# lukeshope/hipims-ocl

Measured on AMD Instinct MI355X. Metric: Mcell-steps/sec fp64 Godunov+HLLC, 4096^2 grid, 1/2/4/8 MI355X; % HBM roofline, higher is better.
Workload: dtype f64

## Files before the change

### hipims-ocl_amd/csrc/hp_domain.hpp

```cpp
#pragma once
#include "../../include/hipims_mi.h"
#include "hp_facts.hpp"
#include "hp_kernels.hpp"
#include "hp_peaks.hpp"
#include "hp_probes.hpp"
#include "hp_zones.hpp"
#include "hp_overview.hpp"
#include "hp_sparse.hpp"
#include "hp_bed.hpp"
#include <rccl/rccl.h>

#include <atomic>
#include <string>
#include <vector>

using namespace hp;

namespace {

thread_local std::string g_last_error;

std::atomic<hp_log_sink_t> g_log_sink{nullptr};
std::atomic<void*>         g_log_user{nullptr};

// ... 130 lines not shown
	void*            saved_scalars = nullptr;
	bool             saved_valid = false;
	ncclComm_t       comm = nullptr;
	int              comm_rank = 0, comm_world = 1;
	hipEvent_t       ev_xchg = nullptr;
	unsigned long long*  peer_mine = nullptr;
	unsigned long long** peer_table = nullptr;
	std::vector<void*>   peer_mapped;
	int              peer_world = 0, peer_rank = 0;
	bool             peer_agreed = false;
	uint64_t         peer_rounds = 0;
	void*            peer_state[2][2] = {{nullptr, nullptr}, {nullptr, nullptr}};
	long             peer_rows[2] = {0, 0};
	unsigned*        push_arrived = nullptr;
	bool             peer_direct = false;
	bool             push_now = false;
	unsigned long long* tail_words = nullptr;
	bool             fill_now = false;
	void*            z_state = nullptr;
	unsigned long long* haz_words = nullptr;
	unsigned         pair_gen = 0;
	void*            still_rec = nullptr;
	size_t           still_rec_slots = 0;
	int              still_rec_half = 0;
	bool             still_rec_last = false;
	uint64_t         pair_cold_starts = 0;
	hipEvent_t       tune_ev[4] = {nullptr, nullptr, nullptr, nullptr};
	int              tune_phase = 0;
	bool             tune_prefer_pairs = true;
	uint64_t         tune_next = 0;
	uint64_t         tune_samples = 0, tune_switches = 0;
	float            tune_pair_ms = 0.f, tune_single_ms = 0.f;
	uint64_t         pairs = 0;
	unsigned         single_streak = 0;
	uint64_t         flux_launches = 0, flux_launches_tailed = 0;
	bool             tail_failed = false;
	bool             strip_first = false;
	bool             tail_allowed = false;
	bool             tail_want = false;
	int              tail_fresh = 0;
	bool             tail_done = false;
	bool             spec_now = false;
	uint32_t         spec_pending = 0;
	void*            spec_state = nullptr;
	void*            spec_scalars = nullptr;
	struct { int adv_fresh; uint64_t cells_calculated, iterations; } spec_host;
	uint64_t         spec_batches = 0, spec_replays = 0;
	OutputStage      out;
// ... 30 lines not shown
```

### hipims-ocl_amd/csrc/hp_engine.hip

```cpp
#include "hp_domain.hpp"
#include "hp_observers.hpp"
#include <hip/hip_ext.h>
#include <dlfcn.h>

#include <algorithm>
#include <cmath>
#include <cstdio>
#include <cstdlib>
#include <cstring>
#include <random>
#include <string>
#include <vector>
#include <unistd.h>

namespace {

constexpr size_t CFL_SLOT_BYTES = 1024;

struct Rccl {
	void* handle = nullptr;
	decltype(&ncclGetUniqueId)   GetUniqueId = nullptr;
	decltype(&ncclCommInitRank)  CommInitRank = nullptr;
	decltype(&ncclCommDestroy)   CommDestroy = nullptr;
	decltype(&ncclGroupStart)    GroupStart = nullptr;
// ... 576 lines not shown
{
	if (d->desc.math_mode == HP_MATH_STRICT) return true;
	static const int forced = std::getenv("HP_PAIR_EXACT") ? (std::atoi(std::getenv("HP_PAIR_EXACT")) != 0 ? 1 : 0) : -1;
	if (forced >= 0) return forced != 0;
	for (const Boundary& b : d->bdy)
		if ((b.kind == 0 && b.definition == HP_UNIFORM_LOSS_RATE) || (b.kind == 1 && b.definition == HP_GRIDDED_MASS_FLUX)) return true;
	return false;
}
static int pair_stamps_alloc(hp_domain* d)
{
	if (!pair_exact(d) || d->z_state) return HP_OK;
	const size_t rec = (size_t)4 * d->esize + 16;
	HIP_TRY(hipMalloc(&d->z_state, d->cells * rec));
	HIP_TRY(hipMalloc((void**)&d->haz_words, 64));
	HIP_TRY(hipMemsetAsync(d->z_state, 0, d->cells * rec, d->stream));
	HIP_TRY(hipMemsetAsync(d->haz_words, 0, 64, d->stream));
	return HP_OK;
}
static bool pair_skip_enabled()
{
	static const bool v = !(std::getenv("HP_PAIR_SKIP") && std::atoi(std::getenv("HP_PAIR_SKIP")) == 0);
	return v;
}
static int still_rec_alloc(hp_domain* d, const int windows)
{
	const size_t slots = (size_t)windows * (size_t)d->desc.rows;
	if (d->still_rec && d->still_rec_slots == slots) return HP_OK;
	hipFree(d->still_rec);
	d->still_rec = nullptr;
	d->facts.buffers_written_outside();
	const size_t bytes = (2 * slots + 1) * sizeof(StillRec);
	HIP_TRY(hipMalloc(&d->still_rec, bytes));
	HIP_TRY(hipMemsetAsync(d->still_rec, 0xff, bytes, d->stream));
	d->still_rec_slots = slots;
	return HP_OK;
}
template <typename T> int pair_cold_start(hp_domain* d)
{
	int rc;
	d->facts.buffers_written_outside();
	if ((rc = apply_boundaries<T>(d, d->state[0])) != HP_OK) return rc;
	if ((rc = launch_reduce<T>(d, d->state[0], d->own_lo, d->own_hi)) != HP_OK) return rc;
	hipLaunchKernelGGL((pair_cold_start_words<T>), dim3(1), dim3(1), 0, d->stream, (T*)d->cfl_slot);
	HIP_TRY(hipGetLastError());
	d->facts.cold_started();
	d->pair_cold_starts++;
	return HP_OK;
}
template <typename T> int run_pair_t(hp_domain* d, const bool strip, const bool followed)
{
	const Params<T> p = make_params<T>(d);
	TileMap tm;
	unsigned blocks;
	long lo, hi;
	if (strip) {
		const bool south = d->desc.row_offset > 0, north = d->desc.row_offset + d->desc.rows < d->desc.global_rows;
		lo = south ? d->ghost_rows : 1;
// ... 11 lines not shown
	const int kind = make_tail<T>(d, blocks, PART_ALL, d->stream, tail_limit(), tail);
	d->tail_want = false; d->tail_allowed = false; d->push_now = false;
	if (kind != (strip ? 2 : 1)) return HP_ERR_STATE;
	const bool bdy = !d->bdy.empty();
	int rc;
	if ((rc = pair_stamps_alloc(d)) != HP_OK) return rc;
	bool in_place = false;
	if (bdy && !d->facts->m1_valid) {
		if ((rc = pair_cold_start<T>(d)) != HP_OK) return rc;
		in_place = true;
	} else if (bdy) in_place = d->facts->pair_fused_next;
	tail.pair = bdy ? 2 : 1;
	tail.bdy_flag = bdy && followed ? 1 : 0;
	PairAux<T> aux{};
	const bool exact = pair_exact(d) && d->z_state != nullptr;
	if (exact) aux.stamps = StampBufs<T>{(char*)d->z_state, d->haz_words};
	aux.prev_gen = d->facts->other_stale ? d->pair_gen : 0u;
	aux.gen = ++d->pair_gen;
	if (aux.gen == 0) aux.gen = ++d->pair_gen;
	aux.list = (const AreaBdyList<T>*)d->fused_list; aux.fuse_next = bdy && followed ? 1 : 0; aux.in_place = in_place ? 1 : 0;
	aux.truncated = (d->desc.quirks & HP_QUIRK_BDY_TRUNCATED) != 0 ? 1 : 0;
	const bool recs = sizeof(T) == 8 && pair_skip_enabled() && !strip && !bdy && !exact && d->desc.math_mode != HP_MATH_STRICT && rseg2 <= 32;
	if (recs) {
		if ((rc = still_rec_alloc(d, tm.nstrips)) != HP_OK) return rc;
		StillRec* const base = (StillRec*)d->still_rec;
		aux.still_out = base + (size_t)(d->still_rec_half ^ 1) * d->still_rec_slots;
		aux.still_in = d->facts->still_rec_valid ? base + (size_t)d->still_rec_half * d->still_rec_slots : nullptr;
		aux.still_rows = d->desc.rows;
	}
	const void* src = d->state[0];
	void* dst = d->state[1];
	const bool sample = d->timing_stride > 0 && d->timing_used < d->timing_events.size() &&
	                    (d->timing_counter++ % (uint64_t)d->timing_stride) == 0;
	if (sample) HIP_TRY(hipEventRecord(d->timing_events[d->timing_used].first, d->stream));
#define HP_LAUNCH_K1B2(CFL_, BDY_, HZ_, TAIL_)                                                                                            \
	hipLaunchKernelGGL((godunov_march2<false, CFL_, BDY_, HZ_, TAIL_, T>), dim3(blocks), dim3(256), 0, d->stream, p, (const Scalars<T>*)d->scalars, \
	                   (const T*)d->bed, (const State4<T>*)src, (State4<T>*)dst, (const T*)d->manning, (T*)d->cfl_slot,                    \
	                   (const T*)d->cfl_slot + SLOT_EDGE, tm, tail, aux)
#define HP_LAUNCH_K1B(CFL_, BDY_, TAIL_) do { if (exact) HP_LAUNCH_K1B2(CFL_, BDY_, true, TAIL_); else HP_LAUNCH_K1B2(CFL_, BDY_, false, TAIL_); } while (0)
	if (d->desc.math_mode == HP_MATH_STRICT)
		hipLaunchKernelGGL((godunov_march2<true, 1, false, true, 1, T>), dim3(blocks), dim3(256), 0, d->stream, p, (const Scalars<T>*)d->scalars,
		                   (const T*)d->bed, (const State4<T>*)src, (State4<T>*)dst, (const T*)d->manning, (T*)d->cfl_slot,
		                   (const T*)d->cfl_slot + SLOT_EDGE, tm, tail, aux);
	else
	if (strip)    { if (d->desc.dynamic_dt) HP_LAUNCH_K1B2(1, false, false, 2); else HP_LAUNCH_K1B2(0, false, false, 2); }
	else if (bdy) HP_LAUNCH_K1B(1, true, 1);
	else          { if (d->desc.dynamic_dt) HP_LAUNCH_K1B(1, false, 1); else HP_LAUNCH_K1B(0, false, 1); }
#undef HP_LAUNCH_K1B
#undef HP_LAUNCH_K1B2
	d->facts.pair_queued(bdy, followed);
	HIP_TRY(hipGetLastError());
// ... 1747 lines not shown
	double total = 0.0;
	uint32_t n = 0;
	for (size_t i = 0; i < d->timing_used; ++i) {
		float ms = 0.f;
		HIP_TRY(hipEventElapsedTime(&ms, d->timing_events[i].first, d->timing_events[i].second));
		total += std::max(0.0, (double)ms - d->timing_overhead_ms);
		++n;
	}
	*avg_ms = n ? total / n : 0.0;
	*samples = n;
	return HP_OK;
}

int hp_pair_stats(hp_domain_t* d, uint64_t out[12])
{
	int rc = check_domain(d);
	if (rc != HP_OK) return rc;
	if (!out) return fail(HP_ERR_INVALID, "out == NULL");
	out[0] = d->pairs; out[1] = d->pair_cold_starts; out[2] = out[3] = 0;
	HIP_TRY(hipStreamSynchronize(d->stream));
	if (tuner_on(d) && (rc = tuner_poll(d)) != HP_OK) return rc;
	out[4] = d->tune_samples; out[5] = d->tune_switches; out[6] = d->tune_prefer_pairs ? 1 : 0;
	out[7] = d->tune_single_ms > 0.f ? (uint64_t)(1000.0 * d->tune_pair_ms / d->tune_single_ms) : 0;
	out[8] = out[9] = out[10] = out[11] = 0;
	if (d->still_rec && d->still_rec_last) {
		const StillRec* half = (const StillRec*)d->still_rec + (size_t)d->still_rec_half * d->still_rec_slots;
		unsigned long long* counts = (unsigned long long*)((StillRec*)d->still_rec + 2 * d->still_rec_slots);
		HIP_TRY(hipMemsetAsync(counts, 0, 16, d->stream));
		hipLaunchKernelGGL(still_rec_count, dim3(256), dim3(256), 0, d->stream, half, d->still_rec_slots, counts);
		HIP_TRY(hipGetLastError());
		unsigned long long host_counts[2] = {0, 0};
		HIP_TRY(hipMemcpyAsync(host_counts, counts, sizeof host_counts, hipMemcpyDeviceToHost, d->stream));
		HIP_TRY(hipStreamSynchronize(d->stream));
		out[9] = host_counts[0]; out[10] = host_counts[1];
	}
	if (d->haz_words) {
		unsigned long long used = 0;
		HIP_TRY(hipMemcpy(&used, d->haz_words + 2, sizeof used, hipMemcpyDeviceToHost));
		out[8] = used;
	}
	if (!d->z_state) return HP_OK;
	unsigned long long* counts = d->haz_words + 4;
	HIP_TRY(hipMemsetAsync(counts, 0, 16, d->stream));
	if (d->desc.precision == 8)
		hipLaunchKernelGGL((stamps_count<double>), dim3(1024), dim3(256), 0, d->stream, StampBufs<double>{(char*)d->z_state, d->haz_words}, d->pair_gen, d->cells, counts);
	else
		hipLaunchKernelGGL((stamps_count<float>), dim3(1024), dim3(256), 0, d->stream, StampBufs<float>{(char*)d->z_state, d->haz_words}, d->pair_gen, d->cells, counts);
	HIP_TRY(hipGetLastError());
	unsigned long long host_counts[2] = {0, 0};
	HIP_TRY(hipMemcpyAsync(host_counts, counts, sizeof host_counts, hipMemcpyDeviceToHost, d->stream));
	HIP_TRY(hipStreamSynchronize(d->stream));
	out[2] = host_counts[0]; out[3] = host_counts[1];
	return HP_OK;
}

int hp_launch_counts(hp_domain_t* d, uint64_t* flux_launches, uint64_t* with_tail)
{
	int rc = check_domain(d);
	if (rc != HP_OK) return rc;
	if (!flux_launches || !with_tail) return fail(HP_ERR_INVALID, "null argument");
	*flux_launches = d->flux_launches;
	*with_tail = d->flux_launches_tailed;
	return HP_OK;
}

int hp_kernel_timing_overhead(hp_domain_t* d, double* overhead_ms)
{
	int rc = check_domain(d);
	if (rc != HP_OK) return rc;
	if (!overhead_ms) return fail(HP_ERR_INVALID, "null argument");
	*overhead_ms = d->timing_overhead_ms;
	return HP_OK;
}

}
```

### hipims-ocl_amd/csrc/hp_kernels.hpp

```cpp
#pragma once

#include "hp_math.hpp"
#include "hp_tiling.hpp"

namespace hp {

template <bool STRICT, typename T>
__global__ __launch_bounds__(256) void godunov_basic(const Params<T> p, const Scalars<T>* __restrict__ sc,
                                                     const T* __restrict__ bed, const State4<T>* __restrict__ src,
                                                     State4<T>* __restrict__ dst, const T* __restrict__ manning,
                                                     const long y_lo, const long y_hi)
{
	const long x = (long)blockIdx.x * blockDim.x + threadIdx.x;
	const long y = (long)blockIdx.y * blockDim.y + threadIdx.y + y_lo;
	if (x >= p.cols - 1 || y >= y_hi || x <= 0) return;
	const size_t id = (size_t)y * p.cols + x;
	const T dt = sc->dt;

	if (dt <= T(0)) { dst[id] = src[id]; return; }

	const State4<T> c = src[id];
	const T zb = bed[id], n = manning[id];
	if (c.zmax <= T(-9999.0) || c.z == T(-9999.0)) { dst[id] = c; return; }

// ... 182 lines not shown
	if (threadIdx.x != 0) return;
	advance_body<UPDATE_ONLY>(p, sc, slot, fresh & 3);
}

template <typename T> struct LaunchTail {
	unsigned long long* done;
	unsigned            flux_blocks;
	int                 pair;
	unsigned long long* done1;
	int                 bdy_flag;
	unsigned            poll_blocks;
	unsigned long long  timeout;
	int                 fresh;
	Scalars<T>*         sc;
	T*                  slot;
	PeerBox             box;
	State4<T>*          peer_rows[2];
	int                 edge_rows[4];
};

#ifndef HP_TAIL_FORMAL_ORDER
#define HP_TAIL_FORMAL_ORDER 0
#endif
template <bool TWO = false, typename T>
__device__ __forceinline__ void tail_block_done(const LaunchTail<T>& tail, const T m, const int wave, const int lane, const long y0, const long y1, const T m1 = T(0))
{
	__shared__ T part[4];
	__shared__ T part1[4];
	const bool sends = (y0 < tail.edge_rows[1] && y1 > tail.edge_rows[0]) || (y0 < tail.edge_rows[3] && y1 > tail.edge_rows[2]);
	if (sends) asm volatile("s_waitcnt vmcnt(0)" ::: "memory");
	if (lane == 0) { part[wave] = m; if (TWO) part1[wave] = m1; }
	__syncthreads();
	bool block_sends = false;
	if (threadIdx.x == 0) {
		block_sends = sends;
		T b = part[0];
		for (int w = 1; w < 4; ++w) if (part[w] > b) b = part[w];
		if (TWO) {
			T b1 = part1[0];
			for (int w = 1; w < 4; ++w) if (part1[w] > b1) b1 = part1[w];
			__hip_atomic_store(tail.done1 + blockIdx.x, peer_bits(b1), __ATOMIC_RELAXED, __HIP_MEMORY_SCOPE_AGENT);
		}
#if HP_TAIL_FORMAL_ORDER
		if (block_sends) __hip_atomic_store(tail.done + blockIdx.x, peer_bits(b), __ATOMIC_RELEASE, __HIP_MEMORY_SCOPE_SYSTEM);
		else
#endif
		__hip_atomic_store(tail.done + blockIdx.x, peer_bits(b), __ATOMIC_RELAXED, __HIP_MEMORY_SCOPE_AGENT);
		(void)block_sends;
	}
}

#ifndef HP_TAIL_POLL_SLEEP
#define HP_TAIL_POLL_SLEEP 1
#endif
template <typename T>
__device__ __forceinline__ void launch_tail(const Params<T>& p, const LaunchTail<T>& tail)
{
	__shared__ T part[4];
// ... 172 lines not shown
}
__device__ __forceinline__ float first_lane(const float v) { return __int_as_float(__builtin_amdgcn_readfirstlane(__float_as_int(v))); }
__device__ __forceinline__ double first_lane(const double v)
{
	return __hiloint2double(__builtin_amdgcn_readfirstlane(__double2hiint(v)), __builtin_amdgcn_readfirstlane(__double2loint(v)));
}
__device__ __forceinline__ unsigned long long value_bits(const double v) { return (unsigned long long)__double_as_longlong(v); }
template <typename V> __device__ __forceinline__ V from_east(const V v) { return lane_move<DPP_WAVE_ROL1>(v); }
template <typename V> __device__ __forceinline__ V from_west(const V v) { return lane_move<DPP_WAVE_ROR1>(v); }

template <typename T> struct RowRegs { State4<T> c; T zb, n; };

template <typename T>
__device__ __forceinline__ Side<T> side_from_east(const Side<T>& s)
{
	Side<T> r;
	r.eta = from_east(s.eta); r.zb = from_east(s.zb);
	r.qx = from_east(s.qx);   r.qy = from_east(s.qy);
	r.u0 = from_east(s.u0);   r.v0 = from_east(s.v0);
	return r;
}


__device__ __forceinline__ bool tile_rows(const TileMap& tm, const int wave, long& strip, long& y0, long& y1)
{
	const unsigned band = blockIdx.x % (unsigned)tm.nbands, i = blockIdx.x / (unsigned)tm.nbands;
	const unsigned nbig_tiles = (unsigned)(tm.groups * tm.nbig);
	const long band_y0 = tm.y_begin + (long)band * tm.band_stride;
	const long band_y1 = (band_y0 + tm.band_rows < tm.y_end) ? (band_y0 + tm.band_rows) : tm.y_end;
	unsigned g;
	long h;
	if (i < nbig_tiles) {
		g = i % (unsigned)tm.groups;
		h = tm.rseg;
		y0 = band_y0 + (long)(i / (unsigned)tm.groups) * tm.rseg;
	} else {
		const unsigned j = i - nbig_tiles;
		g = j % (unsigned)tm.groups;
		h = tm.rseg_tail;
		y0 = band_y0 + (long)tm.nbig * tm.rseg + (long)(j / (unsigned)tm.groups) * tm.rseg_tail;
	}
	y1 = (y0 + h < band_y1) ? (y0 + h) : band_y1;
	strip = (long)g * 4 + wave;
	const bool any = y0 < band_y1 && strip < tm.nstrips;
	if (tm.flip) {
		const long top = band_y0 + (band_y1 - y1);
		y1 = band_y0 + (band_y1 - y0);
		y0 = top;
	}
	return any;
}

template <typename T> struct UniformBdy { const T* series; uint32_t entries; int definition; T interval, length; };
template <typename T> struct GriddedBdy {
	const T* grids; uint64_t entries, grows, gcols; int definition; T resolution, off_x, off_y, interval;
};

template <typename T>
__device__ __forceinline__ bool bdy_in_range(const Params<T>& p, const long x, const long gy, const bool truncated)
{
	if (x >= p.cols - 1 || gy >= p.global_rows - 1 || x <= 0 || gy <= 0) return false;
	if (truncated && (x >= (p.cols / 8) * 8 || gy >= (p.global_rows / 8) * 8)) return false;
	return true;
}

constexpr int AREA_BDY_MAX = 8;
template <typename T> struct AreaBdy {
	int kind;
	UniformBdy<T> u;
	GriddedBdy<T> g;
};
template <typename T> struct AreaBdyList { int count; AreaBdy<T> b[AREA_BDY_MAX]; };


constexpr int FUSED_BDY_MAX = 3;
template <typename T> struct FusedBdy {
	T    inc_lo, inc_hi;
	int  y_switch;
	int  mode;
};

template <typename T> constexpr unsigned stamp_rec() { return (unsigned)sizeof(State4<T>) + 16u; }
template <typename T> struct StampBufs { char* rec; unsigned long long* haz; };
template <typename T> __device__ __forceinline__ unsigned stamp_gen(const StampBufs<T>& b, const size_t id)
{
	return *reinterpret_cast<const unsigned*>(b.rec + id * stamp_rec<T>() + sizeof(State4<T>));
}
template <typename T> __device__ __forceinline__ State4<T> stamp_state(const StampBufs<T>& b, const size_t id)
{
	const T* v = reinterpret_cast<const T*>(b.rec + id * stamp_rec<T>());
	State4<T> c; c.z = v[0]; c.zmax = v[1]; c.qx = v[2]; c.qy = v[3];
	return c;
}
struct StillRec { unsigned long long z, b; unsigned tag, pad[3]; };
constexpr unsigned STILL_TAG_RUN = 1, STILL_TAG_SKIP = 2;
template <typename T> struct PairAux {
	StampBufs<T>          stamps;
	unsigned              gen, prev_gen;
	const AreaBdyList<T>* list;
	int                   fuse_next;
	int                   in_place;
	int                   truncated;
	StillRec*             still_out;
	const StillRec*       still_in;
	long                  still_rows;
};

#ifndef HP_K1_STRICT_WAVES
#define HP_K1_STRICT_WAVES 3
#endif
#ifndef HP_K1_FAST_WAVES
#define HP_K1_FAST_WAVES 3
#endif
#ifndef HP_K1_F32_WAVES
#define HP_K1_F32_WAVES 5
#endif
template <bool STRICT, typename T> constexpr int march_waves() { return sizeof(T) == 4 ? HP_K1_F32_WAVES : (STRICT ? HP_K1_STRICT_WAVES : HP_K1_FAST_WAVES); }

template <bool STRICT, typename T> constexpr int march_waves_max() { return sizeof(T) == 4 ? 8 : march_waves<STRICT, T>(); }
template <bool STRICT, int CFL_MODE, bool FUSED, int TAIL, typename T, bool SPEC = false>
__global__ __launch_bounds__(256) __attribute__((amdgpu_waves_per_eu(march_waves<STRICT, T>(), march_waves_max<STRICT, T>()))) void godunov_march(const Params<T> p, const Scalars<T>* sc,
                                                     const T* __restrict__ bed, const State4<T>* __restrict__ src,
                                                     State4<T>* __restrict__ dst, const T* __restrict__ manning,
                                                     T* cfl_slot, const T* __restrict__ edge_max,
                                                     const TileMap tm, const AreaBdyList<T>* __restrict__ fused_list,
                                                     const int fuse_next, const int flags, const LaunchTail<T> tail)
{
	if (TAIL != 0 && blockIdx.x >= tail.flux_blocks) {
		launch_tail(p, tail);
// ... 310 lines not shown
	}
	if (FUSED && blockIdx.x == 0 && wave == 0 && lane == 0) cfl_slot[SLOT_BDY] = fuse_flag ? T(1) : T(0);
	}
	if (TAIL != 0) tail_block_done(tail, wave_vmax, wave, lane, y0, y1);
}

template <typename T> struct RowU1 { State4<T> c; T zb; bool plain; };

template <bool STRICT, int CFL_MODE, bool BDY, bool HZ, int TAIL, typename T>
#ifndef HP_K1B_WAVES_MIN
#define HP_K1B_WAVES_MIN 3
#endif
#ifndef HP_K1B_F32_WAVES_MIN
#define HP_K1B_F32_WAVES_MIN 5
#endif
#ifndef HP_K1B_F32_WAVES_MAX
#define HP_K1B_F32_WAVES_MAX 5
#endif
__global__ __launch_bounds__(256) __attribute__((amdgpu_waves_per_eu(sizeof(T) == 4 ? (STRICT ? 3 : (HZ ? 4 : HP_K1B_F32_WAVES_MIN)) : (STRICT ? HP_K1B_STRICT_WAVES : HP_K1B_WAVES_MIN), sizeof(T) == 4 ? (STRICT ? 3 : HP_K1B_F32_WAVES_MAX) : (STRICT ? HP_K1B_STRICT_WAVES : 3)))) void godunov_march2(
	const Params<T> p, const Scalars<T>* sc, const T* __restrict__ bed, const State4<T>* __restrict__ src,
	State4<T>* __restrict__ dst, const T* __restrict__ manning, T* cfl_slot, const T* __restrict__ edge_max,
	const TileMap tm, const LaunchTail<T> tail, const PairAux<T> aux)
{
	if (TAIL != 0 && blockIdx.x >= tail.flux_blocks) {
		launch_tail(p, tail);
		return;
	}
	__shared__ T inc_tab[BDY ? 4 * 3 * FUSED_BDY_MAX * 2 * 64 : 1];
	const int lane = threadIdx.x & 63, wave = __builtin_amdgcn_readfirstlane((int)(threadIdx.x >> 6));
	long strip, y0, y1;
	T wave_vmax = T(0), wave_vmax1 = T(0);
	if (tile_rows(tm, wave, strip, y0, y1)) {

	const long x = strip * MARCH2_COLS - 1 + lane;
	const long xc = x < 0 ? 0 : (x < p.cols ? x : (p.cols - 1));
	const bool out_x = lane >= 2 && lane <= MARCH2_COLS + 1 && x <= p.cols - 2;
	const bool ring_x = x <= 0 || x >= p.cols - 1;
	const T vs = p.vs;
	const bool with_friction = p.friction != 0;
	const T inv_dx = STRICT ? p.inv_dx_pow2 : p.inv_dx;

	Scalars<T> s1 = *sc;
	const Scalars<T> s0 = s1;
	const T dt_a = s1.dt;
	advance_scalars(p, s1, p.dynamic_dt ? cfl_slot[BDY ? SLOT_M1 : SLOT_SAVED] : T(0));
	const T dt_b = s1.dt;
	const bool skip_a = dt_a <= T(0), skip_b = dt_b <= T(0);
	constexpr bool SCALAR_CONSTS = !STRICT && sizeof(T) == 8;
	constexpr bool HIDE = BDY || HZ;
	const StepConsts<T> ka{uniform_value<HIDE>(-(dt_a * p.inv_dx)), uniform_value<HIDE>(dt_a * gravity<T>()), SCALAR_CONSTS};
	const StepConsts<T> kb{uniform_value<HIDE>(-(dt_b * p.inv_dx)), uniform_value<HIDE>(dt_b * gravity<T>()), SCALAR_CONSTS};

	const long row_base = y0 - 2 < 0 ? 0 : y0 - 2, col_base = strip * MARCH2_COLS - 1 < 0 ? 0 : strip * MARCH2_COLS - 1;
	const size_t cell0 = (size_t)row_base * p.cols + (size_t)col_base;
	const size_t cells_left = (size_t)p.cols * p.rows - cell0;
// ... 97 lines not shown
					if (b.g.definition == 0) {
						inc_lo = rate_lo / T(3600000.0) * thj[j];
						inc_hi = rate_hi / T(3600000.0) * thj[j];
					} else {
						inc_lo = rate_lo / (p.dx * p.dx) * thj[j];
						inc_hi = rate_hi / (p.dx * p.dx) * thj[j];
					}
					ysw[k] = (int)(row_base + n_lo);
					mode = 2u;
				}
				if (mode == 3u) continue;
				tab[((j * FUSED_BDY_MAX + k) * 2 + 0) * 64 + lane] = inc_lo;
				tab[((j * FUSED_BDY_MAX + k) * 2 + 1) * 64 + lane] = inc_hi;
				modes = (modes & ~(3u << (2 * (j * FUSED_BDY_MAX + k)))) | (mode << (2 * (j * FUSED_BDY_MAX + k)));
				act |= 1u << j;
			}
		}
	}
	const bool fuse = BDY && aux.fuse_next != 0;

	T vmax = T(0), vmax1 = T(0);
	unsigned stale_rows = 0;

	constexpr bool RECS = !STRICT && !BDY && !HZ && TAIL == 1 && sizeof(T) == 8;
	unsigned long long still_kz = 0, still_kb = 0;
	unsigned still_marks = 0;
	auto write_recs = [&](const unsigned tag) {
		if (!RECS || aux.still_out == nullptr) return;
		const __amdgpu_buffer_rsrc_t srd = make_srd(aux.still_out + (size_t)strip * aux.still_rows, (size_t)aux.still_rows * sizeof(StillRec));
		const bool m = lane < 32 && ((still_marks >> (unsigned)lane) & 1u) != 0;
		hp_u32x4 a;
		a.x = m ? (unsigned)still_kz : ~0u; a.y = m ? (unsigned)(still_kz >> 32) : ~0u;
		a.z = m ? (unsigned)still_kb : ~0u; a.w = m ? (unsigned)(still_kb >> 32) : ~0u;
		unsigned voff = lane < y1 - y0 ? (unsigned)((y0 + lane) * (long)sizeof(StillRec)) : HP_OOB;
		asm volatile("" : "+v"(voff));
		store_operands_own(a);
		__builtin_amdgcn_raw_buffer_store_b128(a, srd, (int)voff, 0, 0);
		__builtin_amdgcn_raw_buffer_store_b32(m ? tag : 0u, srd, (int)voff + 16, 0, 0);
		store_fence(a, voff, 0u);
	};
	auto tile_known = [&]() -> bool {
		const long xw = strip * MARCH2_COLS - 1;
		if (xw < 1 || xw + 63 > p.cols - 2 || y0 - 2 < 1 || y1 + 1 > last_row - 1 || y1 - y0 > 32) return false;
		const int nr = (int)(y1 - y0) + 4, n = 3 * nr;
		const __amdgpu_buffer_rsrc_t srd = make_srd(aux.still_in + (size_t)(strip - 1) * aux.still_rows, (size_t)3 * aux.still_rows * sizeof(StillRec));
		auto voff = [&](const int i) {
			const int w = i < nr ? 0 : (i < 2 * nr ? 1 : 2);
// ... 333 lines not shown
				if (TAIL == 2) store_peer(fuse ? next : c, y, true);
				if (CFL_MODE == 1 && (int)y >= tm.price_lo && (int)y < tm.price_hi) {
					const T s = cfl_speed<STRICT>(c.z, c.zmax, c.qx, c.qy, zb, p.qs);
					if (s > vmax) vmax = s;
					if (live2) {
						const T s2 = cfl_speed<STRICT>(next.z, next.zmax, next.qx, next.qy, zb, p.qs);
						if (s2 > vmax1) vmax1 = s2;
					}
				}
			}
		}
	}
	if (!live2) vmax1 = vmax;
	};

	auto raise_word = [&]() { if (hz_on && wave_any(stamped) && lane == 0) aux.stamps.haz[aux.gen & 1u] = (unsigned long long)aux.gen; };
	if (RECS && aux.still_in != nullptr && !skip_a && !skip_b && tile_known()) {
		still_marks = ~0u;
		write_recs(STILL_TAG_SKIP);
		if (CFL_MODE == 1 && out_x && (int)y1 > tm.price_lo && (int)y0 < tm.price_hi)
			vmax = cfl_speed<STRICT>(T(__longlong_as_double((long long)still_kz)), T(0), T(0), T(0), T(__longlong_as_double((long long)still_kb)), p.qs);
		vmax1 = vmax;
	} else {
	if (BDY && act != 0) { if (hz_any) march(std::true_type(), std::true_type()); else march(std::true_type(), std::false_type()); }
	else                 { if (hz_any) march(std::false_type(), std::true_type()); else march(std::false_type(), std::false_type()); }
	raise_word();
	}

	if (CFL_MODE != 0) {
		if (blockIdx.x == 0 && wave == 0) { const T e = *edge_max; if (e > vmax) vmax = e; if (e > vmax1) vmax1 = e; }
		vmax = wave_max(vmax);
		if (BDY) vmax1 = wave_max(vmax1);
		if (TAIL != 0) { wave_vmax = vmax; wave_vmax1 = vmax1; }
		else if (lane == 0 && vmax > T(0)) atomic_max_nonneg(cfl_slot, vmax);
	}
	}
	if (TAIL != 0) tail_block_done<BDY>(tail, wave_vmax, wave, lane, y0, y1, wave_vmax1);
}

template <typename T>
__global__ __launch_bounds__(256) void stamps_to_buffer(State4<T>* __restrict__ other, const StampBufs<T> b, const unsigned gen, const size_t cells)
{
	if (b.haz[gen & 1u] != (unsigned long long)gen) return;
	for (size_t id = (size_t)blockIdx.x * blockDim.x + threadIdx.x; id < cells; id += (size_t)gridDim.x * blockDim.x)
		if (stamp_gen(b, id) == gen) other[id] = stamp_state(b, id);
}

template <typename T>
__global__ __launch_bounds__(256) void stamps_count(const StampBufs<T> b, const unsigned gen, const size_t cells, unsigned long long* counts)
{
	unsigned long long last = 0, any = 0;
	for (size_t id = (size_t)blockIdx.x * blockDim.x + threadIdx.x; id < cells; id += (size_t)gridDim.x * blockDim.x) {
		const unsigned g = stamp_gen(b, id);
		last += (g != 0 && g == gen); any += (g != 0);
	}
	for (int off = 32; off > 0; off >>= 1) { last += __shfl_down(last, off); any += __shfl_down(any, off); }
	if ((threadIdx.x & 63) == 0 && (last | any)) { atomicAdd(counts, last); atomicAdd(counts + 1, any); }
}
__global__ __launch_bounds__(256) void still_rec_count(const StillRec* __restrict__ rec, const size_t n, unsigned long long* counts)
{
// ... 636 lines not shown
```

### hipims-ocl_amd/csrc/hp_tiling.hpp

```cpp
#pragma once
#include <algorithm>
#include <cstdlib>
#include <initializer_list>
#include <vector>

namespace hp {

constexpr int MARCH_COLS = 62;
constexpr int MARCH2_COLS = 60;
constexpr int MUSCL_COLS = 60;

struct TileMap {
	int  nstrips, groups;
	long y_begin, y_end;
	int  nbands;
	long band_stride;
	int  band_rows;
	int  rseg, nbig;
	int  rseg_tail, ntail;
	int  price_lo, price_hi;
	int  flip;
};

struct TilingKnobs {
	bool   rseg_refine = true;
	bool   search = true, search_pair = true;
	bool   search_f32 = false;
	double tiling_fill = 3.5, march2_fill = 4.0;
	int    march_rseg = 0, muscl_rseg = 0, inertial_rseg = 0, march2_rseg = 0;
	int    tail_rseg = 0, tail_pct = -1;
	bool   print_tiling = false;
};
struct LaunchKnobs {
	long   halo_rows = 0;
	int    nbands = 0;
};

struct Tiling {
	int  march_rseg = 16;
	int  muscl_rseg = 32;
	int  inertial_rseg = 32;
	int  march_nbands = 8, muscl_nbands = 8, inertial_nbands = 8;
	int  march_rseg_parts = 16, inertial_rseg_parts = 16;
	int  march2_rseg = 24, march2_nbands = 8;
	bool march2_pays = false;
// ... 183 lines not shown
```

### hipims-ocl_amd/hipims_mi/__init__.py

```python
from __future__ import annotations

import ctypes as C
import os
import weakref

import numpy as np

HERE = os.path.dirname(os.path.abspath(__file__))
PKG_ROOT = os.path.dirname(HERE)
LIB_PATH = os.path.join(PKG_ROOT, "lib", "libhipims_mi.so")

SCHEME_GODUNOV, SCHEME_MUSCL_HANCOCK, SCHEME_INERTIAL = 0, 1, 2
ARRAY_STATE, ARRAY_BED, ARRAY_MANNING = 0, 1, 2
QUIRK_CFL_READS_PRIMARY, QUIRK_BDY_TRUNCATED, QUIRK_MUSCL_NEIGHBOUR_Y_IS_BED, QUIRKS_REFERENCE = 1, 2, 4, 7
MATH_FAST, MATH_STRICT = 0, 1
KERNEL_AUTO, KERNEL_BASIC = 0, 1
UNIFORM_RAIN_INTENSITY, UNIFORM_LOSS_RATE = 0, 1
GRIDDED_RAIN_INTENSITY, GRIDDED_RAIN_ACCUMUL, GRIDDED_MASS_FLUX = 0, 1, 2
DEPTH_IGNORE, DEPTH_IS_FSL, DEPTH_IS_DEPTH, DEPTH_IS_CRITICAL = 0, 1, 2, 3
DISCHARGE_IGNORE, DISCHARGE_IS_DISCHARGE, DISCHARGE_IS_VELOCITY, DISCHARGE_IS_VOLUME = 0, 1, 2, 3
PTR_STATE_NEXT_SRC, PTR_STATE_OTHER, PTR_BED, PTR_MANNING, PTR_CFL_MAX, PTR_SCALARS = range(6)
(OUT_DEPTH, OUT_MAXDEPTH, OUT_FSL, OUT_MAXFSL, OUT_DISCHARGE_X, OUT_DISCHARGE_Y, OUT_VELOCITY_X, OUT_VELOCITY_Y, OUT_FROUDE,
 OUT_COUNT) = range(10)
OUT_CODES = {"depth": OUT_DEPTH, "maxdepth": OUT_MAXDEPTH, "fsl": OUT_FSL, "maxfsl": OUT_MAXFSL, "dischargex": OUT_DISCHARGE_X,
# ... 1 lines not shown
AGG_MAX, AGG_MIN, AGG_COUNT, AGG_KINDS = range(4)
AGG_CODES = {"max": AGG_MAX, "min": AGG_MIN, "count": AGG_COUNT}
OVERVIEW_FACTOR_MAX = 4096
(PEAK_SPEED, PEAK_UNIT_DISCHARGE, PEAK_HAZARD, PEAK_ARRIVAL_TIME, PEAK_WET_DURATION, PEAK_COUNT) = range(6)
PEAK_CODES = {"peakspeed": PEAK_SPEED, "peakunitdischarge": PEAK_UNIT_DISCHARGE, "hazard": PEAK_HAZARD,
              "arrivaltime": PEAK_ARRIVAL_TIME, "wetduration": PEAK_WET_DURATION}
NO_CELL = 2 ** 64 - 1

EXPORTS = [
    "hp_abi_version", "hp_device_count", "hp_device_info", "hp_last_error", "hp_set_log_sink", "hp_domain_desc_default",
    "hp_domain_create", "hp_domain_destroy", "hp_domain_upload", "hp_domain_download", "hp_domain_upload_rows", "hp_state_save", "hp_state_restore",
    "hp_domain_derive", "hp_domain_stats", "hp_overview_shape", "hp_domain_overview", "hp_domain_sparse",
    "hp_peaks_enable", "hp_peaks_disable", "hp_peaks_reset", "hp_peaks_sample", "hp_peaks_read", "hp_peaks_info",
    "hp_probes_enable", "hp_probes_disable", "hp_probes_reset", "hp_probes_sample", "hp_probes_read", "hp_probes_info",
    "hp_zones_enable", "hp_zones_disable", "hp_zones_reset", "hp_zones_sample", "hp_zones_read", "hp_zones_info",
    "hp_bed_shape_add", "hp_bed_shapes_clear", "hp_bed_apply", "hp_bed_info",
    "hp_boundary_add_uniform", "hp_boundary_add_gridded", "hp_boundary_add_cell", "hp_boundary_clear", "hp_boundaries_fused", "hp_set_target_time", "hp_set_time",
    "hp_force_timestep", "hp_reset_counters", "hp_update_timestep", "hp_step_batch", "hp_read_scalars",
    "hp_sync", "hp_is_busy", "hp_step_begin", "hp_step_end", "hp_step_needs_reduction", "hp_device_ptr", "hp_stream", "hp_set_halo_overlap",
    "hp_stream_halo", "hp_comm_load", "hp_comm_unique_id", "hp_strip_comm_init", "hp_strip_step_batch", "hp_strip_update_timestep",
    "hp_strip_comm_destroy", "hp_strip_info", "hp_strip_peer_ticket", "hp_strip_peer_connect", "hp_strip_peer_round",
    "hp_strip_peer_disconnect", "hp_timer_start",
    "hp_timer_stop", "hp_kernel_timing", "hp_kernel_timing_read", "hp_kernel_timing_overhead",
    "hp_launch_counts", "hp_pair_stats",
]


class HipimsError(RuntimeError):
    pass


LOG_SINK = C.CFUNCTYPE(None, C.c_int, C.c_char_p, C.c_void_p)
_log_sink_ref = None


def set_log_sink(callback):
    global _log_sink_ref
    lib = load_library()
    if callback is None:
        sink = C.cast(None, LOG_SINK)
    else:
        sink = LOG_SINK(lambda level, msg, _user: callback(int(level), msg.decode(errors="replace")))
    _check(lib, lib.hp_set_log_sink(sink, None), "hp_set_log_sink")
    _log_sink_ref = sink


class DeviceInfo(C.Structure):
# ... 855 lines not shown
    def kernel_timing(self, stride):
        _check(self.lib, self.lib.hp_kernel_timing(self.h, stride), "hp_kernel_timing")

    def kernel_timing_read(self):
        avg, n = C.c_double(0), C.c_uint32(0)
        _check(self.lib, self.lib.hp_kernel_timing_read(self.h, C.byref(avg), C.byref(n)), "hp_kernel_timing_read")
        return avg.value, n.value

    def launch_counts(self):
        if not hasattr(self.lib, "hp_launch_counts"):
            return None
        a, b = C.c_uint64(0), C.c_uint64(0)
        _check(self.lib, self.lib.hp_launch_counts(self.h, C.byref(a), C.byref(b)), "hp_launch_counts")
        return a.value, b.value

    def pair_stats(self):
        if not hasattr(self.lib, "hp_pair_stats"):
            return None
        out = (C.c_uint64 * 12)()
        self.lib.hp_pair_stats.argtypes = [C.c_void_p, C.POINTER(C.c_uint64)]
        _check(self.lib, self.lib.hp_pair_stats(self.h, out), "hp_pair_stats")
        return dict(pairs=out[0], cold_starts=out[1], stamped_last=out[2], stamped_ever=out[3], tune_samples=out[4],
                    tune_switches=out[5], prefers_pairs=bool(out[6]), pair_over_single=out[7] / 1000.0, stale_used=out[8],
                    skipped_rows=out[9], still_rows=out[10])

    def kernel_timing_overhead(self):
        if not hasattr(self.lib, "hp_kernel_timing_overhead"):
            return 0.0
        ms = C.c_double(0)
        _check(self.lib, self.lib.hp_kernel_timing_overhead(self.h, C.byref(ms)), "hp_kernel_timing_overhead")
        return ms.value

    def depth_velocity(self, state=None, bed=None):
        state = self.download() if state is None else state
        bed = self._bed_host if bed is None else bed
        depth = np.maximum(0.0, state[..., 0].astype(np.float64) - bed.astype(np.float64))
        with np.errstate(divide="ignore", invalid="ignore"):
            u = np.where(depth > 1e-8, state[..., 2] / depth, 0.0)
            v = np.where(depth > 1e-8, state[..., 3] / depth, 0.0)
        return depth, u, v
```

### include/hipims_mi.h

```cpp
#ifndef HIPIMS_MI_H
#define HIPIMS_MI_H

#include <stddef.h>
#include <stdint.h>

#ifdef __cplusplus
extern "C" {
#endif

#define HP_ABI_VERSION 2

typedef enum {
	HP_OK              =  0,
	HP_ERR_INVALID     = -1,
	HP_ERR_NO_DEVICE   = -2,
	HP_ERR_HIP         = -3,
	HP_ERR_UNSUPPORTED = -4,
	HP_ERR_STATE       = -5
} hp_status;

enum { HP_SCHEME_GODUNOV = 0, HP_SCHEME_MUSCL_HANCOCK = 1, HP_SCHEME_INERTIAL = 2 };

enum { HP_ARRAY_STATE = 0, HP_ARRAY_BED = 1, HP_ARRAY_MANNING = 2 };

// ... 234 lines not shown
	int32_t comm_ranks;
	int32_t comm_rank;
	int32_t halo_overlap;
	int32_t ghost_rows;
	int32_t peer_max;
	int32_t peer_halo;
} hp_strip_info_t;
int hp_strip_info(hp_domain_t* d, hp_strip_info_t* out);

#define HP_PEER_TICKET_BYTES 384
int hp_strip_peer_ticket(hp_domain_t* d, void* ticket_out);
int hp_strip_peer_connect(hp_domain_t* d, const void* tickets, int count, int rank, int* active);
int hp_strip_peer_round(hp_domain_t* d, double value, double* max_out);
int hp_strip_peer_disconnect(hp_domain_t* d);

int hp_timer_start(hp_domain_t* d);
int hp_timer_stop(hp_domain_t* d, float* elapsed_ms);
int hp_kernel_timing(hp_domain_t* d, int enable_stride);
int hp_kernel_timing_read(hp_domain_t* d, double* avg_ms, uint32_t* samples);
int hp_kernel_timing_overhead(hp_domain_t* d, double* overhead_ms);
int hp_launch_counts(hp_domain_t* d, uint64_t* flux_launches, uint64_t* with_tail);

int hp_pair_stats(hp_domain_t* d, uint64_t out[12]);

#ifdef __cplusplus
}
#endif
#endif
```

Baseline: 122,600.

## Reorder pair-kernel tiles so blocks that marched last step dispatch first

Each flux block in the paired kernel records whether it did real marching work or skipped via still records, appending its tile id to per-band heavy or light lists. On the next launch, blocks remap their tile index so heavy tiles are scheduled first (in reverse) and light ones after, aiming to reduce tail imbalance when skip-heavy and work-heavy tiles are mixed. This adds atomics per block, extra record storage, and an indirection on tile lookup, and the order is reused only when the tile map matches. A host query API exposes the recorded order.

```diff
diff --git a/hipims-ocl_amd/csrc/hp_domain.hpp b/hipims-ocl_amd/csrc/hp_domain.hpp
--- a/hipims-ocl_amd/csrc/hp_domain.hpp
+++ b/hipims-ocl_amd/csrc/hp_domain.hpp
@@ -176,8 +176,15 @@
 	unsigned         pair_gen = 0;
 	void*            still_rec = nullptr;
 	size_t           still_rec_slots = 0;
+	size_t           still_rec_stride = 0;
 	int              still_rec_half = 0;
 	bool             still_rec_last = false;
+	int              order_nbands = 0;
+	unsigned         order_per_band = 0;
+	uint64_t         order_used = 0;
+	bool             order_valid[2] = {false, false};
+	TileMap          order_tm[2] = {};
+	unsigned         order_blocks[2] = {0, 0};
 	uint64_t         pair_cold_starts = 0;
 	hipEvent_t       tune_ev[4] = {nullptr, nullptr, nullptr, nullptr};
 	int              tune_phase = 0;
diff --git a/hipims-ocl_amd/csrc/hp_engine.hip b/hipims-ocl_amd/csrc/hp_engine.hip
--- a/hipims-ocl_amd/csrc/hp_engine.hip
+++ b/hipims-ocl_amd/csrc/hp_engine.hip
@@ -622,17 +622,27 @@
 	static const bool v = !(std::getenv("HP_PAIR_SKIP") && std::atoi(std::getenv("HP_PAIR_SKIP")) == 0);
 	return v;
 }
-static int still_rec_alloc(hp_domain* d, const int windows)
+static bool pair_order_enabled()
+{
+	static const bool v = pair_skip_enabled() && !(std::getenv("HP_PAIR_ORDER") && std::atoi(std::getenv("HP_PAIR_ORDER")) == 0);
+	return v;
+}
+static int still_rec_alloc(hp_domain* d, const int windows, const int nbands, const unsigned per_band)
 {
 	const size_t slots = (size_t)windows * (size_t)d->desc.rows;
-	if (d->still_rec && d->still_rec_slots == slots) return HP_OK;
+	if (d->still_rec && d->still_rec_slots == slots && d->order_nbands == nbands && d->order_per_band == per_band) return HP_OK;
 	hipFree(d->still_rec);
 	d->still_rec = nullptr;
 	d->facts.buffers_written_outside();
-	const size_t bytes = (2 * slots + 1) * sizeof(StillRec);
+	d->order_valid[0] = d->order_valid[1] = false;
+	const size_t set_recs = pair_order_recs(nbands, per_band), stride = slots + set_recs;
+	const size_t bytes = (2 * stride + 1) * sizeof(StillRec);
 	HIP_TRY(hipMalloc(&d->still_rec, bytes));
 	HIP_TRY(hipMemsetAsync(d->still_rec, 0xff, bytes, d->stream));
-	d->still_rec_slots = slots;
+	for (int h = 0; h < 2; ++h)
+		HIP_TRY(hipMemsetAsync((StillRec*)d->still_rec + (size_t)h * stride + slots, 0, set_recs * sizeof(StillRec), d->stream));
+	d->still_rec_slots = slots; d->still_rec_stride = stride;
+	d->order_nbands = nbands; d->order_per_band = per_band;
 	return HP_OK;
 }
 template <typename T> int pair_cold_start(hp_domain* d)
@@ -690,11 +700,19 @@
 	aux.truncated = (d->desc.quirks & HP_QUIRK_BDY_TRUNCATED) != 0 ? 1 : 0;
 	const bool recs = sizeof(T) == 8 && pair_skip_enabled() && !strip && !bdy && !exact && d->desc.math_mode != HP_MATH_STRICT && rseg2 <= 32;
 	if (recs) {
-		if ((rc = still_rec_alloc(d, tm.nstrips)) != HP_OK) return rc;
+		if ((rc = still_rec_alloc(d, tm.nstrips, tm.nbands, (unsigned)(tm.groups * (tm.nbig + tm.ntail)))) != HP_OK) return rc;
 		StillRec* const base = (StillRec*)d->still_rec;
-		aux.still_out = base + (size_t)(d->still_rec_half ^ 1) * d->still_rec_slots;
-		aux.still_in = d->facts->still_rec_valid ? base + (size_t)d->still_rec_half * d->still_rec_slots : nullptr;
+		aux.still_out = base + (size_t)(d->still_rec_half ^ 1) * d->still_rec_stride;
+		aux.still_in = d->facts->still_rec_valid ? base + (size_t)d->still_rec_half * d->still_rec_stride : nullptr;
 		aux.still_rows = d->desc.rows;
+	}
+	const bool order = recs && pair_order_enabled();
+	if (order) {
+		const int in = d->still_rec_half, out = in ^ 1;
+		aux.order = 1 | (out == 1 ? 4 : 0);
+		if (d->order_valid[in] && d->order_blocks[in] == blocks && same_tile_map(d->order_tm[in], tm)) { aux.order |= 2; d->order_used++; }
+		d->order_valid[in] = false;
+		d->order_valid[out] = true; d->order_tm[out] = tm; d->order_blocks[out] = blocks;
 	}
 	const void* src = d->state[0];
 	void* dst = d->state[1];
@@ -2488,10 +2506,11 @@
 	if (tuner_on(d) && (rc = tuner_poll(d)) != HP_OK) return rc;
 	out[4] = d->tune_samples; out[5] = d->tune_switches; out[6] = d->tune_prefer_pairs ? 1 : 0;
 	out[7] = d->tune_single_ms > 0.f ? (uint64_t)(1000.0 * d->tune_pair_ms / d->tune_single_ms) : 0;
-	out[8] = out[9] = out[10] = out[11] = 0;
+	out[8] = out[9] = out[10] = 0;
+	out[11] = d->order_used;
 	if (d->still_rec && d->still_rec_last) {
-		const StillRec* half = (const StillRec*)d->still_rec + (size_t)d->still_rec_half * d->still_rec_slots;
-		unsigned long long* counts = (unsigned long long*)((StillRec*)d->still_rec + 2 * d->still_rec_slots);
+		const StillRec* half = (const StillRec*)d->still_rec + (size_t)d->still_rec_half * d->still_rec_stride;
+		unsigned long long* counts = (unsigned long long*)((StillRec*)d->still_rec + 2 * d->still_rec_stride);
 		HIP_TRY(hipMemsetAsync(counts, 0, 16, d->stream));
 		hipLaunchKernelGGL(still_rec_count, dim3(256), dim3(256), 0, d->stream, half, d->still_rec_slots, counts);
 		HIP_TRY(hipGetLastError());
@@ -2520,6 +2539,33 @@
 	return HP_OK;
 }
 
+int hp_pair_order(hp_domain_t* d, uint32_t* out, size_t cap, uint64_t info[4])
+{
+	int rc = check_domain(d);
+	if (rc != HP_OK) return rc;
+	if (!info) return fail(HP_ERR_INVALID, "info == NULL");
+	info[0] = info[1] = info[2] = info[3] = 0;
+	const int half = d->still_rec_half;
+	if (!d->still_rec || !d->order_valid[half]) return HP_OK;
+	const TileMap& tm = d->order_tm[half];
+	const unsigned nb = (unsigned)tm.nbands, per_band = (unsigned)(tm.groups * (tm.nbig + tm.ntail));
+	info[0] = nb; info[1] = per_band;
+	if (!out || cap < (size_t)nb * per_band) return HP_OK;
+	std::vector<unsigned> set(pair_order_words((int)nb, per_band));
+	HIP_TRY(hipStreamSynchronize(d->stream));
+	HIP_TRY(hipMemcpy(set.data(), (const StillRec*)d->still_rec + (size_t)half * d->still_rec_stride + d->still_rec_slots, set.size() * sizeof(unsigned),
+	                  hipMemcpyDeviceToHost));
+	for (unsigned band = 0; band < nb; ++band) {
+		const unsigned H = std::min(set[band], per_band);
+		info[3] += H;
+		const unsigned* heavy = set.data() + 2u * nb + (size_t)band * per_band;
+		const unsigned* light = set.data() + 2u * nb + (size_t)(nb + band) * per_band;
+		for (unsigned i = 0; i < per_band; ++i) out[(size_t)band * per_band + i] = ordered_tile(i, H, heavy, light);
+	}
+	info[2] = 1;
+	return HP_OK;
+}
+
 int hp_launch_counts(hp_domain_t* d, uint64_t* flux_launches, uint64_t* with_tail)
 {
 	int rc = check_domain(d);
diff --git a/hipims-ocl_amd/csrc/hp_kernels.hpp b/hipims-ocl_amd/csrc/hp_kernels.hpp
--- a/hipims-ocl_amd/csrc/hp_kernels.hpp
+++ b/hipims-ocl_amd/csrc/hp_kernels.hpp
@@ -228,11 +228,15 @@
 #ifndef HP_TAIL_FORMAL_ORDER
 #define HP_TAIL_FORMAL_ORDER 0
 #endif
-template <bool TWO = false, typename T>
-__device__ __forceinline__ void tail_block_done(const LaunchTail<T>& tail, const T m, const int wave, const int lane, const long y0, const long y1, const T m1 = T(0))
+template <bool TWO = false, bool ORDER = false, typename T>
+__device__ __forceinline__ void tail_block_done(const LaunchTail<T>& tail, const T m, const int wave, const int lane, const long y0, const long y1, const T m1 = T(0),
+                                                const bool marched = false, const unsigned order_tile = 0, unsigned* order_out = nullptr,
+                                                const unsigned nbands = 1, const unsigned per_band = 0)
 {
 	__shared__ T part[4];
 	__shared__ T part1[4];
+	__shared__ int part_marched[4];
+	if constexpr (ORDER) if (lane == 0) part_marched[wave] = marched ? 1 : 0;
 	const bool sends = (y0 < tail.edge_rows[1] && y1 > tail.edge_rows[0]) || (y0 < tail.edge_rows[3] && y1 > tail.edge_rows[2]);
 	if (sends) asm volatile("s_waitcnt vmcnt(0)" ::: "memory");
 	if (lane == 0) { part[wave] = m; if (TWO) part1[wave] = m1; }
@@ -240,6 +244,12 @@
 	bool block_sends = false;
 	if (threadIdx.x == 0) {
 		block_sends = sends;
+		if constexpr (ORDER) if (order_out != nullptr) {
+			const unsigned band = blockIdx.x % nbands;
+			const bool heavy = (part_marched[0] | part_marched[1] | part_marched[2] | part_marched[3]) != 0;
+			const unsigned at = __hip_atomic_fetch_add(order_out + (heavy ? 0u : nbands) + band, 1u, __ATOMIC_RELAXED, __HIP_MEMORY_SCOPE_AGENT);
+			if (at < per_band) order_out[2u * nbands + (heavy ? 0u : nbands * per_band) + band * per_band + at] = order_tile;
+		}
 		T b = part[0];
 		for (int w = 1; w < 4; ++w) if (part[w] > b) b = part[w];
 		if (TWO) {
@@ -458,9 +468,9 @@
 }
 
 
-__device__ __forceinline__ bool tile_rows(const TileMap& tm, const int wave, long& strip, long& y0, long& y1)
-{
-	const unsigned band = blockIdx.x % (unsigned)tm.nbands, i = blockIdx.x / (unsigned)tm.nbands;
+__device__ __forceinline__ bool tile_rows(const TileMap& tm, const int wave, const unsigned i, long& strip, long& y0, long& y1)
+{
+	const unsigned band = blockIdx.x % (unsigned)tm.nbands;
 	const unsigned nbig_tiles = (unsigned)(tm.groups * tm.nbig);
 	const long band_y0 = tm.y_begin + (long)band * tm.band_stride;
 	const long band_y1 = (band_y0 + tm.band_rows < tm.y_end) ? (band_y0 + tm.band_rows) : tm.y_end;
@@ -486,6 +496,10 @@
 	}
 	return any;
 }
+__device__ __forceinline__ bool tile_rows(const TileMap& tm, const int wave, long& strip, long& y0, long& y1)
+{
+	return tile_rows(tm, wave, blockIdx.x / (unsigned)tm.nbands, strip, y0, y1);
+}
 
 template <typename T> struct UniformBdy { const T* series; uint32_t entries; int definition; T interval, length; };
 template <typename T> struct GriddedBdy {
@@ -530,6 +544,8 @@
 }
 struct StillRec { unsigned long long z, b; unsigned tag, pad[3]; };
 constexpr unsigned STILL_TAG_RUN = 1, STILL_TAG_SKIP = 2;
+__device__ __forceinline__ unsigned* pair_order_set(StillRec* still_out, const long still_rows, const int windows, const int nbands, const unsigned per_band,
+                                                    const int order, const bool out);
 template <typename T> struct PairAux {
 	StampBufs<T>          stamps;
 	unsigned              gen, prev_gen;
@@ -537,10 +553,19 @@
 	int                   fuse_next;
 	int                   in_place;
 	int                   truncated;
+	int                   order;
 	StillRec*             still_out;
 	const StillRec*       still_in;
 	long                  still_rows;
 };
+static_assert(sizeof(PairAux<double>) == 72 && sizeof(PairAux<float>) == 72, "PairAux: the order word belongs in the padding");
+__device__ __forceinline__ unsigned* pair_order_set(StillRec* still_out, const long still_rows, const int windows, const int nbands, const unsigned per_band,
+                                                    const int order, const bool out)
+{
+	const size_t slots = (size_t)windows * (size_t)still_rows, stride = slots + pair_order_recs(nbands, per_band);
+	StillRec* const half = out ? still_out : ((order & 4) ? still_out - stride : still_out + stride);
+	return reinterpret_cast<unsigned*>(half + slots);
+}
 
 #ifndef HP_K1_STRICT_WAVES
 #define HP_K1_STRICT_WAVES 3
@@ -897,15 +922,29 @@
 	State4<T>* __restrict__ dst, const T* __restrict__ manning, T* cfl_slot, const T* __restrict__ edge_max,
 	const TileMap tm, const LaunchTail<T> tail, const PairAux<T> aux)
 {
+	constexpr bool RECS = !STRICT && !BDY && !HZ && TAIL == 1 && sizeof(T) == 8;
 	if (TAIL != 0 && blockIdx.x >= tail.flux_blocks) {
 		launch_tail(p, tail);
+		if (RECS && (aux.order & 1) && threadIdx.x < 2u * (unsigned)tm.nbands) {
+			const unsigned pb = (unsigned)(tm.groups * (tm.nbig + tm.ntail));
+			pair_order_set(aux.still_out, aux.still_rows, tm.nstrips, tm.nbands, pb, aux.order, false)[threadIdx.x] = 0u;
+		}
 		return;
 	}
 	__shared__ T inc_tab[BDY ? 4 * 3 * FUSED_BDY_MAX * 2 * 64 : 1];
 	const int lane = threadIdx.x & 63, wave = __builtin_amdgcn_readfirstlane((int)(threadIdx.x >> 6));
 	long strip, y0, y1;
 	T wave_vmax = T(0), wave_vmax1 = T(0);
-	if (tile_rows(tm, wave, strip, y0, y1)) {
+	const unsigned per_band = (unsigned)(tm.groups * (tm.nbig + tm.ntail));
+	auto own_tile = [&]() -> unsigned {
+		const unsigned nb = (unsigned)tm.nbands, band = blockIdx.x % nb, i = blockIdx.x / nb;
+		if (!RECS || !(aux.order & 2)) return i;
+		const unsigned* const in = pair_order_set(aux.still_out, aux.still_rows, tm.nstrips, tm.nbands, per_band, aux.order, false);
+		const unsigned H = in[band] < per_band ? in[band] : per_band;
+		return ordered_tile(i, H, in + 2u * nb + band * per_band, in + 2u * nb + (nb + band) * per_band);
+	};
+	bool marched = false;
+	if (tile_rows(tm, wave, own_tile(), strip, y0, y1)) {
 
 	const long x = strip * MARCH2_COLS - 1 + lane;
 	const long xc = x < 0 ? 0 : (x < p.cols ? x : (p.cols - 1));
@@ -1049,7 +1088,6 @@
 	T vmax = T(0), vmax1 = T(0);
 	unsigned stale_rows = 0;
 
-	constexpr bool RECS = !STRICT && !BDY && !HZ && TAIL == 1 && sizeof(T) == 8;
 	unsigned long long still_kz = 0, still_kb = 0;
 	unsigned still_marks = 0;
 	auto write_recs = [&](const unsigned tag) {
@@ -1429,6 +1467,7 @@
 			vmax = cfl_speed<STRICT>(T(__longlong_as_double((long long)still_kz)), T(0), T(0), T(0), T(__longlong_as_double((long long)still_kb)), p.qs);
 		vmax1 = vmax;
 	} else {
+	marched = true;
 	if (BDY && act != 0) { if (hz_any) march(std::true_type(), std::true_type()); else march(std::true_type(), std::false_type()); }
 	else                 { if (hz_any) march(std::false_type(), std::true_type()); else march(std::false_type(), std::false_type()); }
 	raise_word();
@@ -1442,7 +1481,9 @@
 		else if (lane == 0 && vmax > T(0)) atomic_max_nonneg(cfl_slot, vmax);
 	}
 	}
-	if (TAIL != 0) tail_block_done<BDY>(tail, wave_vmax, wave, lane, y0, y1, wave_vmax1);
+	if (TAIL != 0) tail_block_done<BDY, RECS>(tail, wave_vmax, wave, lane, y0, y1, wave_vmax1, marched, RECS ? own_tile() : 0u,
+	                                                      RECS && (aux.order & 1) ? pair_order_set(aux.still_out, aux.still_rows, tm.nstrips, tm.nbands, per_band, aux.order, true) : nullptr,
+	                                                      (unsigned)tm.nbands, per_band);
 }
 
 template <typename T>
diff --git a/hipims-ocl_amd/csrc/hp_tiling.hpp b/hipims-ocl_amd/csrc/hp_tiling.hpp
--- a/hipims-ocl_amd/csrc/hp_tiling.hpp
+++ b/hipims-ocl_amd/csrc/hp_tiling.hpp
@@ -3,6 +3,12 @@
 #include <cstdlib>
 #include <initializer_list>
 #include <vector>
+
+#ifdef __HIPCC__
+#define HP_TILING_HD __host__ __device__
+#else
+#define HP_TILING_HD
+#endif
 
 namespace hp {
 
@@ -21,6 +27,20 @@
 	int  price_lo, price_hi;
 	int  flip;
 };
+
+inline bool same_tile_map(const TileMap& a, const TileMap& b)
+{
+	return a.nstrips == b.nstrips && a.groups == b.groups && a.y_begin == b.y_begin && a.y_end == b.y_end && a.nbands == b.nbands &&
+	       a.band_stride == b.band_stride && a.band_rows == b.band_rows && a.rseg == b.rseg && a.nbig == b.nbig && a.rseg_tail == b.rseg_tail &&
+	       a.ntail == b.ntail && a.price_lo == b.price_lo && a.price_hi == b.price_hi && a.flip == b.flip;
+}
+
+HP_TILING_HD inline unsigned ordered_tile(const unsigned i, const unsigned H, const unsigned* heavy, const unsigned* light)
+{
+	return i < H ? heavy[H - 1u - i] : light[i - H];
+}
+HP_TILING_HD inline size_t pair_order_words(const int nbands, const unsigned per_band) { return (size_t)2 * (size_t)nbands * ((size_t)per_band + 1); }
+HP_TILING_HD inline size_t pair_order_recs(const int nbands, const unsigned per_band) { return (pair_order_words(nbands, per_band) * 4 + 31) / 32; }
 
 struct TilingKnobs {
 	bool   rseg_refine = true;
diff --git a/hipims-ocl_amd/hipims_mi/__init__.py b/hipims-ocl_amd/hipims_mi/__init__.py
--- a/hipims-ocl_amd/hipims_mi/__init__.py
+++ b/hipims-ocl_amd/hipims_mi/__init__.py
@@ -47,7 +47,7 @@
     "hp_strip_comm_destroy", "hp_strip_info", "hp_strip_peer_ticket", "hp_strip_peer_connect", "hp_strip_peer_round",
     "hp_strip_peer_disconnect", "hp_timer_start",
     "hp_timer_stop", "hp_kernel_timing", "hp_kernel_timing_read", "hp_kernel_timing_overhead",
-    "hp_launch_counts", "hp_pair_stats",
+    "hp_launch_counts", "hp_pair_stats", "hp_pair_order",
 ]
 
 
@@ -949,7 +949,20 @@
         _check(self.lib, self.lib.hp_pair_stats(self.h, out), "hp_pair_stats")
         return dict(pairs=out[0], cold_starts=out[1], stamped_last=out[2], stamped_ever=out[3], tune_samples=out[4],
                     tune_switches=out[5], prefers_pairs=bool(out[6]), pair_over_single=out[7] / 1000.0, stale_used=out[8],
-                    skipped_rows=out[9], still_rows=out[10])
+                    skipped_rows=out[9], still_rows=out[10], ordered_launches=out[11])
+
+    def pair_order(self):
+        if not hasattr(self.lib, "hp_pair_order"):
+            return None
+        self.lib.hp_pair_order.argtypes = [C.c_void_p, C.POINTER(C.c_uint32), C.c_size_t, C.POINTER(C.c_uint64)]
+        info = (C.c_uint64 * 4)()
+        _check(self.lib, self.lib.hp_pair_order(self.h, None, 0, info), "hp_pair_order")
+        if not info[0] * info[1]:
+            return dict(valid=0, nbands=int(info[0]), per_band=int(info[1]), heavy=0, order=None)
+        order = np.empty((int(info[0]), int(info[1])), np.uint32)
+        _check(self.lib, self.lib.hp_pair_order(self.h, order.ctypes.data_as(C.POINTER(C.c_uint32)), order.size, info), "hp_pair_order")
+        valid = int(info[2])
+        return dict(valid=valid, nbands=int(info[0]), per_band=int(info[1]), heavy=int(info[3]), order=order if valid else None)
 
     def kernel_timing_overhead(self):
         if not hasattr(self.lib, "hp_kernel_timing_overhead"):
diff --git a/include/hipims_mi.h b/include/hipims_mi.h
--- a/include/hipims_mi.h
+++ b/include/hipims_mi.h
@@ -280,6 +280,7 @@
 int hp_launch_counts(hp_domain_t* d, uint64_t* flux_launches, uint64_t* with_tail);
 
 int hp_pair_stats(hp_domain_t* d, uint64_t out[12]);
+int hp_pair_order(hp_domain_t* d, uint32_t* out, size_t cap, uint64_t info[4]);
 
 #ifdef __cplusplus
 }
```

Result: faster. 125,300, median of 6 (+2.2%).
